# BerkIGuler/AdaFortiTran

Hardware: AMD Instinct MI355X
Metric: OFDM frames/sec (120x14 grid, batch 128) + channel-estimation MSE vs reference (higher is better)
Workload: dtype f32; 1 GPU; C3: AdaFortiTran default config (6 layers, d=128, 4 heads, adaptive tokens), 120x14 grid, pilots 12x2; 128 frames per GPU per step; step = model(pilots_cpu, meta_cpu) through the module surface + device MSE partial; value = SURVEY 8(d)'s metric: H2D of pilots + meta INSIDE the step, output left on the device (= value_h2d_inclusive); the bare engine call on inputs resident in HBM is value_resident;; frames_per_gpu=128, global_batch=128, parallelism=frames sharded over 1 rank(s), lanes=1

## Files before the change

### adafortitran_amd/csrc/aft_api.hip

```cpp
#include <algorithm>
#include <atomic>
#include <cstdlib>
#include <cstdarg>
#include <cstdio>
#include <cstring>
#include <mutex>
#include <string>
#include <vector>

#include "aft_internal.h"

namespace aft {

static thread_local char g_err[512] = "";

void set_error(const char *fmt, ...) {
    va_list ap;
    va_start(ap, fmt);
    vsnprintf(g_err, sizeof(g_err), fmt, ap);
    va_end(ap);
}

int hip_fail(const char *what, hipError_t e) {
    set_error("%s: %s", what, hipGetErrorString(e));
// ... 320 lines not shown
            hit->used = false;
        }
        return nullptr;
    }
    ++hit->in_use;
    hit->tick = ++g_lane_tick;
    return &hit->ls;
}
static void release_lane_streams(LaneStreams *ls) {
    if (ls == nullptr) return;
    std::lock_guard<std::mutex> lock(g_lane_mu);
    for (auto &en : g_lane_cache)
        if (&en.ls == ls) { --en.in_use; return; }
}

enum ChainPos { kChainFirst, kChainMiddle, kChainLast };
static ChainFusion chain_fusion_for(ChainPos pos, const aft_config &c, const WeightsDev &w, const Workspace &ws, float *base) {
    ChainFusion f{};
    f.x_blocked = true;
    if (pos == kChainFirst) {
        f.conv_enhanced = base + ws.conv_enhanced;
        f.tokens6 = c.adaptive ? base + ws.tokens6 : nullptr;
        f.lin1_w = w.lin1_w; f.lin1_b = w.lin1_b; f.pos = w.pos;
    } else if (pos == kChainLast) {
        f.lin2_w = w.lin2_w; f.lin2_b = w.lin2_b; f.out6 = base + ws.out6;
    }
    return f;
}

static int run_encoder(const aft_config &c, const WeightsDev &w, const aft_layer_weights *layers, const Workspace &ws, float *base, float *x,
                       int first_layer, int last_layer, hipStream_t st, bool fused = false, const float *prepacked = nullptr,
                       float *x_pt = nullptr, float *vt2 = nullptr) {
    float *attn = base + ws.attn, *q = base + ws.q, *k = base + ws.k, *vt = base + ws.vt;
    const int rows = ws.planes * ws.tokens;
    const size_t pl = packed_layer_floats(c.model_dim);
    const float *wp = prepacked != nullptr ? prepacked : base + ws.wpack;
    if (prepacked == nullptr)
        STEP("pack_weights", launch_pack_weights(c, layers + first_layer, base + ws.wpack + first_layer * pl, last_layer - first_layer + 1, st));
    const ChainFusion first = chain_fusion_for(kChainFirst, c, w, ws, base), middle = chain_fusion_for(kChainMiddle, c, w, ws, base),
                      last = chain_fusion_for(kChainLast, c, w, ws, base);
    if (fused && x_pt != nullptr && x == base + ws.x && first_layer == 0 && last_layer == c.num_layers - 1 &&
        layer_fused_selected(c, ws.planes / 2)) {
        x = x_pt;
        float *kbuf[2] = {k, attn}, *vbuf[2] = {vt, vt2};
        STEP("chain(qkv, plane tiles)", launch_chain_plane_tiles(c, &layers[0], wp, x, q, kbuf[0], vbuf[0], ws.planes, ws.tokens, ws.tokpad, st, &first));
        for (int l = 0; l <= last_layer; ++l) {
            const bool more = l < last_layer;
            STEP("layer", launch_layer(c, &layers[l], wp + l * pl, more ? &layers[l + 1] : nullptr, more ? wp + (l + 1) * pl : nullptr, x, q,
                                       kbuf[l & 1], vbuf[l & 1], kbuf[(l + 1) & 1], vbuf[(l + 1) & 1], ws.planes, ws.tokens, ws.tokpad, st,
                                       more ? &middle : &last));
        }
        return AFT_OK;
    }
    STEP("chain(qkv)", launch_chain(c, nullptr, nullptr, &layers[first_layer], wp + first_layer * pl, nullptr, x, q, k, vt, rows,
                                    ws.tokens, ws.tokpad, st, fused ? &first : nullptr));
// ... 126 lines not shown
    for (int i = 0; i < kMaxLanes; ++i) {
        frames[i] = i < lp.lanes ? lp.frames[i] : 0;
        offset_bytes[i] = i < lp.lanes ? lp.ws_off[i] * sizeof(float) : 0;
    }
    return AFT_OK;
}

static int forward_lane(const aft_config *cfg, const aft_weights *w, const float *prepacked, const float *pilots, const float *snr,
                        const float *ds, const float *dop, float *out, float *base, int batch, hipStream_t st, float *x_pt, float *vt2) {
    const Workspace ws = plan_workspace(*cfg, batch);
    const bool general = !packed_engine_ok(*cfg);
    const WeightsDev wd = weights_window(*w, 0, cfg->num_layers);
    float *wpack = prepacked != nullptr || general ? nullptr : base + ws.wpack;
    float *lent = x_holds_planes(*cfg, ws) ? base + ws.x : nullptr;
    float *up_planes = prologue_upsample_ok(*cfg, wd) ? lent : nullptr;
    STEP("prologue(adapter + pack_weights + upsampler product)",
         launch_prologue(*cfg, wd, snr, ds, dop, base + ws.tokens6, batch, wpack, pilots, up_planes, st, base + ws.convfrag));
    if (wpack != nullptr && cfg->num_layers > kLayerWindow)
        STEP("pack_weights(layers beyond the prologue's window)",
             launch_pack_weights(*cfg, w->layers + kLayerWindow, wpack + packed_layer_floats(cfg->model_dim) * kLayerWindow,
                                 cfg->num_layers - kLayerWindow, st));
    STEP("upsample", launch_upsample(*cfg, wd, pilots, base + ws.conv_enhanced, batch, st, lent, up_planes != nullptr, base + ws.convfrag));
    const int rc = general ? run_encoder_general(*cfg, wd, w->layers, ws, base, batch, st)
                           : run_encoder(*cfg, wd, w->layers, ws, base, base + ws.x, 0, cfg->num_layers - 1, st, true,
                                         prepacked != nullptr ? prepacked : wpack, x_pt, vt2);
    if (rc != AFT_OK) return rc;
    STEP("tail", launch_tail(*cfg, wd, nullptr, base + ws.conv_enhanced, out, batch, st, base + ws.out6, base + ws.convfrag + kConvFragFloats));
    return AFT_OK;
}

static int forward_impl(const aft_config *cfg, const aft_weights *w, const float *prepacked, const float *pilots,
                        const float *snr, const float *ds, const float *dop, float *out, void *workspace,
                        size_t workspace_bytes, int batch, void *stream) {
    int rc = check_config(cfg);
    if (rc != AFT_OK) return rc;
    AFT_REQUIRE(w && pilots && out && workspace, "NULL pointer argument");
    AFT_REQUIRE(batch > 0, "batch must be positive (got %d)", batch);
    AFT_REQUIRE(batch <= max_batch_of(*cfg), "batch %d exceeds aft_max_batch = %d for this configuration (32-bit buffer "
                "offsets: no workspace region may reach 2 GiB); split the batch", batch, max_batch_of(*cfg));
    AFT_REQUIRE(!cfg->adaptive || (snr && ds && dop), "meta_data is required when channel adaptation is enabled");
// ... 210 lines not shown
    AFT_REQUIRE(batch <= max_batch_of(*cfg), "batch %d exceeds aft_max_batch = %d", batch, max_batch_of(*cfg));
    if (!packed_engine_ok(*cfg)) {
        set_error("aft_profile_kernel_f32 replays the packed engine's kernel classes; this configuration runs the general engine");
        return AFT_ERR_SHAPE;
    }
    const Workspace ws = plan_workspace(*cfg, batch);
    AFT_REQUIRE(workspace_bytes >= ws.total * sizeof(float), "workspace too small");
    const WeightsDev wd = weights_window(*w, 0, cfg->num_layers);
    AFT_REQUIRE(cfg->num_layers >= 2 || which != AFT_KERNEL_CHAIN, "chain profile needs >= 2 layers");
    hipStream_t st = static_cast<hipStream_t>(stream);
    float *base = static_cast<float *>(workspace);
    float *x = base + ws.x, *attn = base + ws.attn, *q = base + ws.q, *k = base + ws.k, *vt = base + ws.vt;
    const int rows = ws.planes * ws.tokens;
    float *lent = x_holds_planes(*cfg, ws) ? x : nullptr;
    const float *wp = base + ws.wpack;
    const ChainFusion first = chain_fusion_for(kChainFirst, *cfg, wd, ws, base), middle = chain_fusion_for(kChainMiddle, *cfg, wd, ws, base),
                      last = chain_fusion_for(kChainLast, *cfg, wd, ws, base);
    hipError_t e = hipSuccess;
    for (int i = 0; i < reps && e == hipSuccess; ++i) {
        switch (which) {
            case AFT_KERNEL_UPSAMPLE:
                AFT_REQUIRE(out != nullptr, "upsample profile needs the pilots pointer in `out`");
                e = launch_upsample(*cfg, wd, out, base + ws.conv_enhanced, batch, st, lent, prologue_upsample_ok(*cfg, wd), base + ws.convfrag);
                break;
            case AFT_KERNEL_EMBED:
                e = launch_embed(*cfg, wd, base + ws.conv_enhanced, cfg->adaptive ? base + ws.tokens6 : nullptr, x, batch, st);
                break;
            case AFT_KERNEL_QKV:
                e = launch_chain(*cfg, nullptr, nullptr, &w->layers[0], wp, nullptr, x, q, k, vt, rows, ws.tokens, ws.tokpad, st, &first);
                break;
            case AFT_KERNEL_ATTENTION:
                e = launch_attention(*cfg, q, k, vt, w->layers[0].in_proj_b, attn, ws.planes, ws.tokens, ws.tokpad, st);
                break;
            case AFT_KERNEL_CHAIN:
                e = launch_chain(*cfg, &w->layers[0], wp, &w->layers[1], wp + packed_layer_floats(cfg->model_dim), attn, x, q, k, vt, rows,
                                 ws.tokens, ws.tokpad, st, &middle);
                break;
            case AFT_KERNEL_CHAIN_LAST:
                e = launch_chain(*cfg, &w->layers[0], wp, nullptr, nullptr, attn, x, q, k, vt, rows, ws.tokens, ws.tokpad, st, &last);
                break;
            case AFT_KERNEL_PROLOGUE: {
                AFT_REQUIRE(out != nullptr, "prologue profile needs the pilots pointer in `out`");
                const float *cond = out + (size_t)batch * cfg->pilot_scs * cfg->pilot_symbols * 2;
                e = launch_prologue(*cfg, wd, cond, cond + batch, cond + 2 * batch, base + ws.tokens6, batch, base + ws.wpack, out,
                                    prologue_upsample_ok(*cfg, wd) && !switch_on(SW_PROLOGUE_NO_UP) ? lent : nullptr, st,
                                    base + ws.convfrag);
                break;
            }
            case AFT_KERNEL_TAIL:
                AFT_REQUIRE(out != nullptr, "tail profile needs an output buffer");
                e = launch_tail(*cfg, wd, nullptr, base + ws.conv_enhanced, out, batch, st, base + ws.out6, base + ws.convfrag + kConvFragFloats);
                break;
            default:
                set_error("unknown kernel id %d", which);
                return AFT_ERR_ARG;
        }
    }
    return e == hipSuccess ? AFT_OK : hip_fail("profile", e);
}

}
// ... 1 lines not shown
```

### adafortitran_amd/csrc/aft_internal.h

```cpp
#pragma once

#include <hip/hip_runtime.h>

#include <cstddef>
#include <cstdint>

#include "../../include/adafortitran_amd.h"
#include "switches.h"
#ifdef AFT_DIAG_STAMPS
#include "stamp_report.h"
#endif

namespace aft {

using f32x2 = __attribute__((ext_vector_type(2))) float;
using f32x4 = __attribute__((ext_vector_type(4))) float;
using f32x16 = __attribute__((ext_vector_type(16))) float;

constexpr int kWave = 64;
constexpr int kHeadDim = 32;
constexpr int kTile = 32;
constexpr int kMaxPatchFeatures = 16;

inline __host__ __device__ int round_up(int v, int m) { return (v + m - 1) / m * m; }
// ... 174 lines not shown
    unsigned long long *dev_ = nullptr;
    std::vector<unsigned long long> host_;
    StampKind kind_;
    long long rows_;
    hipStream_t st_;
};
#endif

constexpr size_t kConvFragFloats = 22 * 64 * 4 + 160;
hipError_t launch_upsample(const aft_config &c, const WeightsDev &w, const float *pilots,
                           float *conv_enhanced, int batch, hipStream_t st, float *scratch_planes = nullptr, bool planes_ready = false,
                           const float *conv_frag = nullptr);
hipError_t launch_adapter(const aft_config &c, const WeightsDev &w, const float *snr, const float *ds,
                          const float *dop, float *tokens6, int batch, hipStream_t st);
bool prologue_upsample_ok(const aft_config &c, const WeightsDev &w);
hipError_t launch_prologue(const aft_config &c, const WeightsDev &w, const float *snr, const float *ds, const float *dop,
                           float *tokens6, int batch, float *packed, const float *pilots, float *up_planes, hipStream_t st,
                           float *conv_frag = nullptr);
hipError_t launch_embed(const aft_config &c, const WeightsDev &w, const float *conv_enhanced,
                        const float *tokens6, float *x, int batch, hipStream_t st);
constexpr int kMaxPatchGeneral = 32;
hipError_t launch_embed_any(const aft_config &c, const WeightsDev &w, const float *conv_enhanced,
                            const float *tokens6, float *x, int batch, hipStream_t st);
struct ChainFusion {
    const float *conv_enhanced = nullptr, *tokens6 = nullptr, *lin1_w = nullptr, *lin1_b = nullptr, *pos = nullptr;
    const float *lin2_w = nullptr, *lin2_b = nullptr;
    float *out6 = nullptr;
    bool x_blocked = false;
};
inline int out6_stride(const aft_config &c) { return round_up(c.patch_scs * c.patch_symbols, 8); }
hipError_t launch_chain(const aft_config &c, const aft_layer_weights *mlp_w, const float *mlp_packed,
                        const aft_layer_weights *qkv_w, const float *qkv_packed, const float *attn, float *x,
                        float *q, float *k, float *vt, int rows, int tokens, int tokpad, hipStream_t st,
                        const ChainFusion *fuse = nullptr);
size_t packed_layer_floats(int d);
bool layer_fused_ok(const aft_config &c);
hipError_t launch_chain_plane_tiles(const aft_config &c, const aft_layer_weights *qkv_w, const float *qkv_packed, float *x, float *q,
                                    float *k, float *vt, int planes, int tokens, int tokpad, hipStream_t st, const ChainFusion *fuse);
hipError_t launch_layer(const aft_config &c, const aft_layer_weights *mlp_w, const float *mlp_packed, const aft_layer_weights *qkv_w,
                        const float *qkv_packed, float *x, float *q, const float *k_in, const float *vt_in, float *k_out, float *vt_out,
                        int planes, int tokens, int tokpad, hipStream_t st, const ChainFusion *fuse);
hipError_t launch_pack_weights(const aft_config &c, const aft_layer_weights *layers, float *packed, int count, hipStream_t st);
// ... 143 lines not shown
```

### adafortitran_amd/csrc/chain_device.h

```cpp
#pragma once
#include "aft_internal.h"
#include "srd.h"
#include "stamps.h"

namespace aft {

template <int D>
struct ChainShape {
    static constexpr int WAVES = D / 32;
    static constexpr int THREADS = 64 * WAVES;
    static constexpr int XB = WAVES * 1024;
    static constexpr int HB = 2 * WAVES * 1024;
    static constexpr int ST = 32 * WAVES * 2;
    static constexpr int PAR = 4 * D;
    static constexpr size_t LDS_BYTES = sizeof(float) * (size_t)(XB + HB + ST + PAR);
};

struct ChainArgs {
    const float *attn;
    float *x;
    const float *wo, *w1, *w2, *wqkv;
    const float *bo, *b1, *b2, *g1, *be1, *g2, *be2;
    const float *bv;
    float *q, *k, *vt;
    int rows, tokens, tokpad, heads;
    int x_blocked;
    const float *lin2_w, *lin2_b;
    float *out6;
    int out6_features, out6_stride;
    const float *emb_conv, *emb_tok6, *emb_w1, *emb_b1, *emb_pos;
    int emb_S, emb_T, emb_p0, emb_p1, emb_K;
    unsigned long long *stamps;
    int tpp;
};

ChainArgs make_chain_args(const aft_config &c, const aft_layer_weights *mlp_w, const float *mlp_packed, const aft_layer_weights *qkv_w,
                          const float *qkv_packed, const float *attn, float *x, float *q, float *k, float *vt, int rows, int tokens,
                          int tokpad, const ChainFusion *fuse);

template <int NT, int PFS>
struct WRing {
    f32x4 b[PFS + 1][NT];
};


template <int NKB, int NT, int PFS, int TS>
// ... 152 lines not shown
    const Srd srd_q = make_srd(a.q), srd_k = make_srd(a.k), srd_vt = make_srd(a.vt);
    const unsigned wo_off = (unsigned)w * W * 1024 + lane * 4, w1_off = (unsigned)(2 * w) * W * 1024 + lane * 4;
    const unsigned w2_off = (unsigned)w * (2 * W) * 1024 + lane * 4;
    const unsigned wq_off = (unsigned)w * W * 1024 + lane * 4;
    const Srd srd_bv = make_srd(a.bv);

    if constexpr (MLP) {
        for (int i = tid; i < D; i += S::THREADS) {
            par[i] = a.g1[i];
            par[D + i] = a.be1[i];
            par[2 * D + i] = a.g2[i];
            par[3 * D + i] = a.be2[i];
        }
        __syncthreads();
    }
    constexpr int kEmbSteps = (kMaxPatchFeatures + 6 + 1) / 2;
    float *emb_w = hb + S::XB;
    int *emb_offs = reinterpret_cast<int *>(emb_w + D * (kMaxPatchFeatures + 6));
    if constexpr (!MLP) {
        if (a.emb_conv != nullptr) {
            const int pk = a.emb_p0 * a.emb_p1;
            for (int i = tid; i < D * a.emb_K; i += S::THREADS) emb_w[i] = a.emb_w1[i];
            for (int k = tid; k < a.emb_K; k += S::THREADS)
                emb_offs[k] = k < pk ? (k / a.emb_p1) * a.emb_T + k % a.emb_p1 : ~(k - pk);
            __syncthreads();
        }
    }
    const int ntiles = (a.rows + 31) / 32;
    const int rounds = (tile_end - first_tile + tile_stride - 1) / tile_stride;
    int round = 0;
#ifndef AFT_CHAIN_PFK
// ... 55 lines not shown
            for (int j = 0; j < 4; ++j) emb_acc0[4 * s + j] = b[j] + ps[j];
        }
#pragma unroll
        for (int st = 0; st < kEmbSteps; ++st) {
            const int k = 2 * st + h;
            emb_bv[st] = 0.f;
            if (k < a.emb_K) {
                const int off = emb_offs[k];
                emb_bv[st] = off >= 0 ? cplane[off] : t6[~off];
            }
        }
    };
    if constexpr (!MLP) {
        if (a.emb_conv != nullptr && first_tile < tile_end) emb_request(first_tile);
    }
    int pending_row0 = -1, pending_valid = 0;
    auto reduce_out6 = [&]() {
        const int P = a.out6_features;
        if (PT ? r < pending_valid : pending_row0 + r < a.rows) {
#pragma unroll
            for (int half = 0; half < 2; ++half) {
                const int f0 = 8 * half + 4 * h;
                if (f0 < P) {
                    f32x4 sum = *reinterpret_cast<const f32x4 *>(hb + lane * 8 + 4 * half);
#pragma unroll
                    for (int u = 1; u < W; ++u) {
                        const f32x4 t = *reinterpret_cast<const f32x4 *>(hb + (u * 64 + lane) * 8 + 4 * half);
                        sum += t;
                    }
#pragma unroll
// ... 43 lines not shown
                   w1_lane = ((PT && MLP ? (unsigned)(2 * w) * W * 1024 : w1_off) + lo_lane) * 4,
                   w2_lane = ((PT && MLP ? (unsigned)w * (2 * W) * 1024 : w2_off) + lo_lane) * 4,
                   wq_lane = ((PT && MLP ? (unsigned)w * W * 1024 : wq_off) + lo_lane) * 4;
    AFT_STAMP(tid == 0, a.stamps, tile, 0);
    AFT_STAMP_WALL(tid == 0, a.stamps, tile, 12);
    AFT_STAMP_VALUE(tid == 0, a.stamps, tile, 14, ((unsigned long long)__builtin_amdgcn_s_getreg((4 << 0) | (0 << 6) | (31 << 11)) << 32) |
                                                      __builtin_amdgcn_s_getreg((20 << 0) | (0 << 6) | (31 << 11)));
#ifndef AFT_CHAIN_PFS
#define AFT_CHAIN_PFS 4
#endif
    constexpr int PFD = AFT_CHAIN_PFS, PFF = (AFT_CHAIN_PFS + 1) / 2, PFQ = (AFT_CHAIN_PFS + 2) / 3;
    WRing<1, PFD> ring_d;
    WRing<2, PFF> ring_ff;
    WRing<3, PFQ> ring_qkv;
    f32x16 cur;
    if constexpr (MLP) {
        f32x16 acc_o[1] = {bias_acc(srd_bo, fb, h)};
        gemm_preload<W, 1, PFD, 1>(ring_d, srd_wo, wo_lane);
        if constexpr (PT) {
            request_x_pt(tile, valid_pt);
        } else {
            request_attn(tile, AHEAD ? PFK : 0, W);
            if (!AHEAD) request_x(tile);
        }
        AFT_STAMP(tid == 0, a.stamps, tile, 1);
        if constexpr (BS)
            gemm_run_bs<W, 1, PFD, 1, 0>(ring_d, srd_wo, wo_lane, acc_o, [&](int kb, int m) { return bs_split(of[kb][2 * m], of[kb][2 * m + 1]); });
        else if constexpr (PT)
            gemm_run<W, 1, PFD, 1, 0>(ring_d, srd_wo, wo_lane, acc_o, [&](int kb, int s) {
                return *reinterpret_cast<const f32x4 *>(hb + S::XB + (kb * 4 + s) * 256 + lane * 4);
// ... 80 lines not shown
            }
        }
        if (store_x && row_ok) {
            if (blocked) {
                const unsigned xblk = ((unsigned)row0 * D + w * 1024 + lane * 4) * 4;
#pragma unroll
                for (int s = 0; s < 4; ++s)
                    srd_store(srd_x, xblk + 1024 * s, f32x4{cur[4 * s], cur[4 * s + 1], cur[4 * s + 2], cur[4 * s + 3]});
            } else {
#pragma unroll
                for (int s = 0; s < 4; ++s)
                    srd_store(srd_x, xrow + 32 * s, f32x4{cur[4 * s], cur[4 * s + 1], cur[4 * s + 2], cur[4 * s + 3]});
            }
        }
    } else {
        gemm_preload<W, 3, PFQ, W>(ring_qkv, srd_wq, wq_lane);
        if (a.emb_conv == nullptr) {
            if (!AHEAD) request_x(tile);
#pragma unroll
            for (int s = 0; s < 4; ++s)
#pragma unroll
                for (int j = 0; j < 4; ++j) cur[4 * s + j] = xres[s][j];
        } else {
            f32x16 acc0 = emb_acc0;
            float av[kEmbSteps];
#pragma unroll
            for (int st = 0; st < kEmbSteps; ++st) {
                const int k = 2 * st + h;
                av[st] = k < a.emb_K ? emb_w[(fb + r) * a.emb_K + k] : 0.f;
            }
#pragma unroll
            for (int st = 0; st < kEmbSteps; ++st)
                if (2 * st < a.emb_K) acc0 = __builtin_amdgcn_mfma_f32_32x32x2f32(av[st], emb_bv[st], acc0, 0, 0, 0);
            cur = acc0;
            if (row_ok) {
                if (blocked) {
                    const unsigned xblk = ((unsigned)row0 * D + w * 1024 + lane * 4) * 4;
#pragma unroll
                    for (int s = 0; s < 4; ++s)
                        srd_store(srd_x, xblk + 1024 * s, f32x4{cur[4 * s], cur[4 * s + 1], cur[4 * s + 2], cur[4 * s + 3]});
                } else {
#pragma unroll
                    for (int s = 0; s < 4; ++s)
                        srd_store(srd_x, xrow + 32 * s, f32x4{cur[4 * s], cur[4 * s + 1], cur[4 * s + 2], cur[4 * s + 3]});
                }
            }
        }
    }

    if constexpr (QKV) {
        const float bias_v = __builtin_bit_cast(float, __builtin_amdgcn_raw_buffer_load_b32(srd_bv, (unsigned)(fb + r) * 4, 0, 0));
        float *xq = xb;
        if constexpr (!MLP) xq = (round & 1) ? hb : xb;
        if constexpr (BS) {
            bs_publish(xq, w, lane, cur);
        } else {
#pragma unroll
            for (int s = 0; s < 4; ++s)
                *reinterpret_cast<f32x4 *>(xq + (w * 4 + s) * 256 + lane * 4) = f32x4{cur[4 * s], cur[4 * s + 1], cur[4 * s + 2], cur[4 * s + 3]};
        }
        __syncthreads();
        AFT_STAMP(tid == 0, a.stamps, tile, 9);
        f32x16 vinit;
#pragma unroll
        for (int e = 0; e < 16; ++e) vinit[e] = bias_v;
        f32x16 acc[3];
        acc[2] = vinit;
        if constexpr (BS) {
            acc[0] = bias_acc(make_srd(a.bv - 2 * D), fb, h);
            auto xq_bs = [&](int kb, int m) { return bs_fetch(xq, kb, m, lane); };
            gemm_run_bs<W, 3, PFQ, W, 0x4, decltype(xq_bs), 0x2>(ring_qkv, srd_wq, wq_lane, acc, xq_bs);
        } else {
            auto xq_frag = [&](int kb, int s) { return *reinterpret_cast<const f32x4 *>(xq + (kb * 4 + s) * 256 + lane * 4); };
            gemm_run<W, 3, PFQ, W, 0x4, decltype(xq_frag), 0x3>(ring_qkv, srd_wq, wq_lane, acc, xq_frag);
        }
        AFT_STAMP(tid == 0, a.stamps, tile, 10);
        if (AHEAD && tile + tile_stride < ntiles) request_tile(tile + tile_stride);
        if constexpr (!MLP) {
            if (a.emb_conv != nullptr && tile + tile_stride < tile_end) emb_request(tile + tile_stride);
        }
        if constexpr (PT) {
            const unsigned ph_base = (unsigned)(plane_pt * a.heads + w) * ((unsigned)a.tokpad * kHeadDim) + (unsigned)qt_pt * 1024;
            if (row_ok) {
#pragma unroll
                for (int s = 0; s < 4; ++s) {
                    srd_store(srd_q, (ph_base + lane * 4 + s * 256) * 4, f32x4{acc[0][4 * s], acc[0][4 * s + 1], acc[0][4 * s + 2], acc[0][4 * s + 3]});
                    srd_store(srd_k, (ph_base + lane * 4 + s * 256) * 4, f32x4{acc[1][4 * s], acc[1][4 * s + 1], acc[1][4 * s + 2], acc[1][4 * s + 3]});
                }
            }
#pragma unroll
// ... 150 lines not shown
```

### adafortitran_amd/csrc/k_chain.hip

```cpp
#include <algorithm>
#include <cstdlib>

#include "chain_device.h"
#include "pack_device.h"

#ifndef AFT_CHAIN_MANY_MAX_D
#define AFT_CHAIN_MANY_MAX_D 96
#endif

namespace aft {

template <int D, int ACT, bool MLP, bool QKV>
__global__ __launch_bounds__(D * 2, D <= 128 ? 3 : 2) void chain_kernel(const ChainArgs a) {
    extern __shared__ __attribute__((aligned(16))) float smem[];
    chain_body<D, ACT, MLP, QKV>(a, smem, threadIdx.x, blockIdx.x, gridDim.x, (a.rows + 31) / 32);
}


template <int D, int ACT, bool MLP, bool QKV>
__global__ __launch_bounds__(D * 2, D <= 128 ? 3 : 2) void chain_split_kernel(const ChainArgs a) {
    extern __shared__ __attribute__((aligned(16))) float smem[];
    chain_body<D, ACT, MLP, QKV, true>(a, smem, threadIdx.x, blockIdx.x, gridDim.x, (a.rows + 31) / 32);
}

// ... 77 lines not shown
ChainArgs make_chain_args(const aft_config &c, const aft_layer_weights *m, const float *m_packed, const aft_layer_weights *qw,
                          const float *q_packed, const float *attn, float *x, float *q, float *k, float *vt, int rows, int tokens,
                          int tokpad, const ChainFusion *fuse) {
    const size_t dd = (size_t)c.model_dim * c.model_dim;
    ChainArgs a{};
    if (fuse != nullptr && fuse->out6 != nullptr && m != nullptr && qw == nullptr) {
        a.lin2_w = fuse->lin2_w; a.lin2_b = fuse->lin2_b; a.out6 = fuse->out6;
        a.out6_features = c.patch_scs * c.patch_symbols;
        a.out6_stride = out6_stride(c);
    }
    if (fuse != nullptr && fuse->conv_enhanced != nullptr && m == nullptr) {
        a.emb_conv = fuse->conv_enhanced; a.emb_tok6 = fuse->tokens6; a.emb_w1 = fuse->lin1_w; a.emb_b1 = fuse->lin1_b;
        a.emb_pos = fuse->pos;
        a.emb_S = c.num_scs; a.emb_T = c.num_symbols; a.emb_p0 = c.patch_scs; a.emb_p1 = c.patch_symbols;
        a.emb_K = c.patch_scs * c.patch_symbols + (fuse->tokens6 ? 6 : 0);
    }
    a.attn = attn;
    a.x = x;
    a.x_blocked = fuse != nullptr && fuse->x_blocked ? 1 : 0;
    if (m != nullptr) {
        a.wo = m_packed + 3 * dd; a.bo = m->out_proj_b;
        a.w1 = m_packed + 4 * dd; a.b1 = m->lin1_b;
        a.w2 = m_packed + 6 * dd; a.b2 = m->lin2_b;
        a.g1 = m->norm1_w; a.be1 = m->norm1_b;
        a.g2 = m->norm2_w; a.be2 = m->norm2_b;
    }
    if (qw != nullptr) {
        a.wqkv = q_packed;
        a.bv = qw->in_proj_b + 2 * c.model_dim;
    }
// ... 37 lines not shown
```

### adafortitran_amd/csrc/k_misc.hip

```cpp
#include <algorithm>

#include "aft_internal.h"
#include "conv_device.h"
#include "pack_device.h"

namespace aft {

struct AdapterArgs {
    const float *cond[3];
    const float *w[3][3], *b[3][3];
    float *tokens6;
    int h0, h1, h2, tokens;
};

__device__ __forceinline__ void adapter_body(const AdapterArgs &a, int b, int e, float *sm) {
    float *a0 = sm, *a1 = sm + a.h0;
    const int tid = threadIdx.x;
    const float x = a.cond[e][b];
    constexpr int kH0Max = 8, kPer2 = 3;
    const bool fast = a.h0 <= kH0Max && a.h1 == 42 && a.h2 <= kPer2 * 256 && a.h1 <= 256;
    if (fast) {
        float w0 = 0.f, b0 = 0.f, w1[kH0Max], b1 = 0.f, b2[kPer2];
        f32x2 w2[kPer2][21];
        if (tid < a.h0) { w0 = a.w[e][0][tid]; b0 = a.b[e][0][tid]; }
// ... 61 lines not shown
    for (int e = 0; e < 3; ++e)
        for (int j = 0; j < 3; ++j) { a.w[e][j] = w.ada_w[e][j]; a.b[e][j] = w.ada_b[e][j]; }
    a.tokens6 = tokens6;
    a.h0 = c.hidden[0]; a.h1 = c.hidden[1]; a.h2 = c.hidden[2];
    a.tokens = (c.num_scs / c.patch_scs) * (c.num_symbols / c.patch_symbols);
    return a;
}

hipError_t launch_adapter(const aft_config &c, const WeightsDev &w, const float *snr, const float *ds,
                          const float *dop, float *tokens6, int batch, hipStream_t st) {
    const AdapterArgs a = adapter_args(c, w, snr, ds, dop, tokens6);
    hipLaunchKernelGGL(adapter_kernel, dim3(batch, 3), dim3(256), sizeof(float) * (a.h0 + a.h1), st, a);
    return hipGetLastError();
}

struct PrologueArgs {
    AdapterArgs ad;
    float *packed;
    const float *pilots;
    float *up_planes;
    int adapter_blocks, pack_blocks, d, num_layers, split;
    int up_bx, npix, pf, nplanes;
    float *conv_frag;
    int frag_blocks;
};

__global__ __launch_bounds__(256) void prologue_kernel(const WeightsDev w, const PrologueArgs a) {
    extern __shared__ __attribute__((aligned(16))) float sm[];
    int blk = blockIdx.x;
    if (blk < a.adapter_blocks) {
        adapter_body(a.ad, blk / 3, blk % 3, sm);
        return;
    }
    blk -= a.adapter_blocks;
    if (blk < a.pack_blocks) {
        pack_weights_vec(w, a.packed, a.d, 0, a.num_layers, a.split, (size_t)blk * 256 + threadIdx.x);
        return;
    }
    blk -= a.pack_blocks;
    if (blk < a.frag_blocks) {
        const int v = blk * 256 + threadIdx.x;
        constexpr int kPerStack = kFragFloats / 4;
        if (v < 2 * kPerStack) {
            const int stack = v / kPerStack, rem = v - stack * kPerStack;
            const float *const *cw = stack ? w.ref_w : w.enh_w;
            const float *const *cb = stack ? w.ref_b : w.enh_b;
            f32x4 o;
            if (rem < kFragQuads * 64) {
                const int quad = rem >> 6, lane = rem & 63;
#pragma unroll
                for (int jj = 0; jj < 4; ++jj) o[jj] = conv_frag16_entry(cw[1], cb[1], cw[2], cb[2], 4 * quad + jj, lane);
// ... 4 lines not shown
            }
            *reinterpret_cast<f32x4 *>(a.conv_frag + (size_t)v * 4) = o;
        }
        return;
    }
    blk -= a.frag_blocks;
    upsample_planes_body(sm, w.up_w, w.up_b, a.pilots, a.up_planes, a.npix, a.pf, a.nplanes, blk % a.up_bx, blk / a.up_bx);
}

bool prologue_upsample_ok(const aft_config &c, const WeightsDev &w) {
    return upsample_planes_ok(w.up_w, c.pilot_scs * c.pilot_symbols);
}

hipError_t launch_prologue(const aft_config &c, const WeightsDev &w, const float *snr, const float *ds, const float *dop,
                           float *tokens6, int batch, float *packed, const float *pilots, float *up_planes, hipStream_t st,
                           float *conv_frag) {
    PrologueArgs a{};
    if (conv_frag != nullptr) {
        a.conv_frag = conv_frag;
        a.frag_blocks = (2 * (kFragFloats / 4) + 255) / 256;
    }
    size_t lds = 0;
    if (c.adaptive) {
        a.ad = adapter_args(c, w, snr, ds, dop, tokens6);
        a.adapter_blocks = 3 * batch;
        lds = sizeof(float) * (a.ad.h0 + a.ad.h1);
    }
    if (packed != nullptr) {
        a.packed = packed; a.d = c.model_dim; a.num_layers = std::min(c.num_layers, kLayerWindow);
        a.split = c.precision == AFT_PRECISION_BF16X3 ? 1 : 0;
        a.pack_blocks = (int)((packed_layer_floats(c.model_dim) * a.num_layers / 4 + 255) / 256);
    }
    int up_blocks = 0;
    if (up_planes != nullptr && prologue_upsample_ok(c, w)) {
        a.pilots = pilots; a.up_planes = up_planes;
        a.npix = c.num_scs * c.num_symbols; a.pf = c.pilot_scs * c.pilot_symbols; a.nplanes = 2 * batch;
        a.up_bx = (a.npix + kUpPix - 1) / kUpPix;
        up_blocks = a.up_bx * ((a.nplanes + kUpPlanes - 1) / kUpPlanes);
        lds = std::max(lds, upsample_planes_lds(a.pf));
    }
    const int blocks = a.adapter_blocks + a.pack_blocks + a.frag_blocks + up_blocks;
    if (blocks == 0) return hipSuccess;
    hipLaunchKernelGGL(prologue_kernel, dim3(blocks), dim3(256), lds, st, w, a);
    return hipGetLastError();
}

struct EmbedArgs {
    const float *conv_enhanced, *tokens6, *w1, *b1, *pos;
    float *x;
    int S, T, p0, p1, tokens, d, din, planes;
};

template <int D, bool ADAPTIVE, int PMAX>
__global__ __launch_bounds__(256) void embed_kernel(const EmbedArgs a) {
    constexpr int PER = D / 32, NF = ADAPTIVE ? PMAX + 6 : PMAX;
    const int tid = threadIdx.x, hw = tid >> 5, lane32 = tid & 31;
// ... 392 lines not shown
```

### adafortitran_amd/csrc/switches.h

```cpp
#pragma once

#define AFT_SWITCHES(X) \
    X(LANES, "AFT_LANES", "1 = never split a forward into lanes; 2 .. 4 = always that many shares (header section \"Lanes\")") \
    X(LAYER_FUSED, "AFT_LAYER_FUSED", "0 = never the one-launch-per-layer sequence (k_layer.hip), 1 = wherever its shape is covered (default: where plane-aligned tiles add no round)") \
    X(PROLOGUE_NO_UP, "AFT_PROLOGUE_NO_UP", "measurement: the profiled prologue launch without the pilot upsampler product") \
    X(CONV_NSPLIT, "AFT_CONV_NSPLIT", "1 | 2 | 4 column ranges per plane in the streaming conv kernels (default: by the batch)") \
    X(CONV_BANDED, "AFT_CONV_BANDED", "the banded conv kernel instead of the column- / row-streaming ones") \
    X(CONV_COLUMN_TILES, "AFT_CONV_COLUMN_TILES", "the column-tiled conv path even where a band plan fits; n > 2 = at least n tiles per plane") \
    X(GEMM_BM, "AFT_GEMM_BM", "64 | 96: row tile of the training GEMM (default: by the shape)") \
    X(EMBED_ANY_OLD, "AFT_EMBED_ANY_OLD", "the general engine's own embedding kernel instead of the training path's") \
    X(EMBED_BWD_GENERIC, "AFT_EMBED_BWD_GENERIC", "the vector embedding backward instead of the MFMA one (model_dim 128)") \
    X(TRAIN_UNFUSED_FWD, "AFT_TRAIN_UNFUSED_FWD", "the launch sequence the fused forward chain of a training layer replaced") \
    X(TRAIN_UNFUSED_BWD, "AFT_TRAIN_UNFUSED_BWD", "the launch sequence the fused backward chain of a training layer replaced") \
    X(TRAIN_ATTN_BWD_SPLIT, "AFT_TRAIN_ATTN_BWD_SPLIT", "the two-pass attention backward instead of the one-pass kernel") \
    X(ATTN_BWD_GROUPS, "AFT_ATTN_BWD_GROUPS", "1 | 4 problems per workgroup of the one-pass attention backward (default: by shape)") \
    X(STAMPS, "AFT_STAMPS", "phase stamps printed on the host: the diag variant only (libaft_hip_diag.so, build.build_diag(): -DAFT_DIAG_STAMPS)") \
    X(ALLOW_COMPOSITE, "AFT_ALLOW_COMPOSITE", "1 = run a configuration the kernels do not cover on the PyTorch-ROCm composite") \
    X(TRAIN_NO_FUSED_ENDS, "AFT_TRAIN_NO_FUSED_ENDS", "training: PyTorch's unfold / cat / add around the dense ends, not fused") \
    X(TRAIN_NO_QKV_CHAIN, "AFT_TRAIN_NO_QKV_CHAIN", "training: every layer runs its own in-projection GEMM (no chained tapes)") \
    X(PRECISION, "AFT_PRECISION", "f32 | bf16x3: the estimators' default hip_precision") \
    X(ENCODER_PATH, "AFT_ENCODER_PATH", "auto | launches | plane: aft_config.encoder_path of every HipEngine (`plane`: retired, runs the launches)")

namespace aft {

// ... 12 lines not shown
```

Baseline: 84990 frames/s.

## Fold layer-0 key/value projection through the embedding into prologue tables

Layer 0's K and V projections are rewritten algebraically: since x0 = W1·features + b1 + pos, K/V = (Wkv·W1)·features + (Wkv·(b1+pos)+bv). The prologue now precomputes per-token bias tables and the folded Wkv·W1 matrices, so the first chain kernel computes K and V with a K-deep MFMA (patch features + 6) instead of a model_dim-deep GEMM, leaving only Q on the full product. This adds work and LDS use to the prologue launch and changes the floating-point summation order for layer-0 keys and values.

```diff
diff --git a/adafortitran_amd/csrc/aft_api.hip b/adafortitran_amd/csrc/aft_api.hip
--- a/adafortitran_amd/csrc/aft_api.hip
+++ b/adafortitran_amd/csrc/aft_api.hip
@@ -358,6 +358,14 @@
         if (&en.ls == ls) { --en.in_use; return; }
 }
 
+static bool l0_fold_selected(const aft_config &c) {
+    return packed_engine_ok(c) && c.precision == AFT_PRECISION_F32 && switch_int(SW_L0_FOLD, 1) != 0;
+}
+static L0Fold l0_fold_at(const aft_config &c, const Workspace &ws, float *base) {
+    float *tables = base + ws.attn;
+    return L0Fold{tables, tables + (size_t)ws.tokpad * c.model_dim, base + ws.wpack + (size_t)c.model_dim * c.model_dim};
+}
+
 enum ChainPos { kChainFirst, kChainMiddle, kChainLast };
 static ChainFusion chain_fusion_for(ChainPos pos, const aft_config &c, const WeightsDev &w, const Workspace &ws, float *base) {
     ChainFusion f{};
@@ -374,15 +382,18 @@
 
 static int run_encoder(const aft_config &c, const WeightsDev &w, const aft_layer_weights *layers, const Workspace &ws, float *base, float *x,
                        int first_layer, int last_layer, hipStream_t st, bool fused = false, const float *prepacked = nullptr,
-                       float *x_pt = nullptr, float *vt2 = nullptr) {
+                       float *x_pt = nullptr, float *vt2 = nullptr, const L0Fold *fold = nullptr) {
     float *attn = base + ws.attn, *q = base + ws.q, *k = base + ws.k, *vt = base + ws.vt;
     const int rows = ws.planes * ws.tokens;
     const size_t pl = packed_layer_floats(c.model_dim);
     const float *wp = prepacked != nullptr ? prepacked : base + ws.wpack;
     if (prepacked == nullptr)
         STEP("pack_weights", launch_pack_weights(c, layers + first_layer, base + ws.wpack + first_layer * pl, last_layer - first_layer + 1, st));
-    const ChainFusion first = chain_fusion_for(kChainFirst, c, w, ws, base), middle = chain_fusion_for(kChainMiddle, c, w, ws, base),
-                      last = chain_fusion_for(kChainLast, c, w, ws, base);
+    ChainFusion first = chain_fusion_for(kChainFirst, c, w, ws, base);
+    const ChainFusion middle = chain_fusion_for(kChainMiddle, c, w, ws, base), last = chain_fusion_for(kChainLast, c, w, ws, base);
+    if (fused && fold != nullptr && first_layer == 0) {
+        first.fold_tk = fold->tk; first.fold_tvt = fold->tvt; first.fold_w = fold->wf;
+    }
     if (fused && x_pt != nullptr && x == base + ws.x && first_layer == 0 && last_layer == c.num_layers - 1 &&
         layer_fused_selected(c, ws.planes / 2)) {
         x = x_pt;
@@ -539,8 +550,11 @@
     float *wpack = prepacked != nullptr || general ? nullptr : base + ws.wpack;
     float *lent = x_holds_planes(*cfg, ws) ? base + ws.x : nullptr;
     float *up_planes = prologue_upsample_ok(*cfg, wd) ? lent : nullptr;
+    const bool fold_on = l0_fold_selected(*cfg);
+    const L0Fold fold = fold_on ? l0_fold_at(*cfg, ws, base) : L0Fold{};
     STEP("prologue(adapter + pack_weights + upsampler product)",
-         launch_prologue(*cfg, wd, snr, ds, dop, base + ws.tokens6, batch, wpack, pilots, up_planes, st, base + ws.convfrag));
+         launch_prologue(*cfg, wd, snr, ds, dop, base + ws.tokens6, batch, wpack, pilots, up_planes, st, base + ws.convfrag,
+                         fold_on ? &fold : nullptr));
     if (wpack != nullptr && cfg->num_layers > kLayerWindow)
         STEP("pack_weights(layers beyond the prologue's window)",
              launch_pack_weights(*cfg, w->layers + kLayerWindow, wpack + packed_layer_floats(cfg->model_dim) * kLayerWindow,
@@ -548,7 +562,7 @@
     STEP("upsample", launch_upsample(*cfg, wd, pilots, base + ws.conv_enhanced, batch, st, lent, up_planes != nullptr, base + ws.convfrag));
     const int rc = general ? run_encoder_general(*cfg, wd, w->layers, ws, base, batch, st)
                            : run_encoder(*cfg, wd, w->layers, ws, base, base + ws.x, 0, cfg->num_layers - 1, st, true,
-                                         prepacked != nullptr ? prepacked : wpack, x_pt, vt2);
+                                         prepacked != nullptr ? prepacked : wpack, x_pt, vt2, fold_on ? &fold : nullptr);
     if (rc != AFT_OK) return rc;
     STEP("tail", launch_tail(*cfg, wd, nullptr, base + ws.conv_enhanced, out, batch, st, base + ws.out6, base + ws.convfrag + kConvFragFloats));
     return AFT_OK;
@@ -789,8 +803,11 @@
     const int rows = ws.planes * ws.tokens;
     float *lent = x_holds_planes(*cfg, ws) ? x : nullptr;
     const float *wp = base + ws.wpack;
-    const ChainFusion first = chain_fusion_for(kChainFirst, *cfg, wd, ws, base), middle = chain_fusion_for(kChainMiddle, *cfg, wd, ws, base),
-                      last = chain_fusion_for(kChainLast, *cfg, wd, ws, base);
+    ChainFusion first = chain_fusion_for(kChainFirst, *cfg, wd, ws, base);
+    const ChainFusion middle = chain_fusion_for(kChainMiddle, *cfg, wd, ws, base), last = chain_fusion_for(kChainLast, *cfg, wd, ws, base);
+    const bool fold_on = l0_fold_selected(*cfg);
+    const L0Fold fold = fold_on ? l0_fold_at(*cfg, ws, base) : L0Fold{};
+    if (fold_on) { first.fold_tk = fold.tk; first.fold_tvt = fold.tvt; first.fold_w = fold.wf; }
     hipError_t e = hipSuccess;
     for (int i = 0; i < reps && e == hipSuccess; ++i) {
         switch (which) {
@@ -819,7 +836,7 @@
                 const float *cond = out + (size_t)batch * cfg->pilot_scs * cfg->pilot_symbols * 2;
                 e = launch_prologue(*cfg, wd, cond, cond + batch, cond + 2 * batch, base + ws.tokens6, batch, base + ws.wpack, out,
                                     prologue_upsample_ok(*cfg, wd) && !switch_on(SW_PROLOGUE_NO_UP) ? lent : nullptr, st,
-                                    base + ws.convfrag);
+                                    base + ws.convfrag, fold_on ? &fold : nullptr);
                 break;
             }
             case AFT_KERNEL_TAIL:
diff --git a/adafortitran_amd/csrc/aft_internal.h b/adafortitran_amd/csrc/aft_internal.h
--- a/adafortitran_amd/csrc/aft_internal.h
+++ b/adafortitran_amd/csrc/aft_internal.h
@@ -212,9 +212,13 @@
 hipError_t launch_adapter(const aft_config &c, const WeightsDev &w, const float *snr, const float *ds,
                           const float *dop, float *tokens6, int batch, hipStream_t st);
 bool prologue_upsample_ok(const aft_config &c, const WeightsDev &w);
+constexpr int kFoldSteps = (kMaxPatchFeatures + 6 + 1) / 2;
+struct L0Fold {
+    float *tk, *tvt, *wf;
+};
 hipError_t launch_prologue(const aft_config &c, const WeightsDev &w, const float *snr, const float *ds, const float *dop,
                            float *tokens6, int batch, float *packed, const float *pilots, float *up_planes, hipStream_t st,
-                           float *conv_frag = nullptr);
+                           float *conv_frag = nullptr, const L0Fold *fold = nullptr);
 hipError_t launch_embed(const aft_config &c, const WeightsDev &w, const float *conv_enhanced,
                         const float *tokens6, float *x, int batch, hipStream_t st);
 constexpr int kMaxPatchGeneral = 32;
@@ -224,6 +228,7 @@
     const float *conv_enhanced = nullptr, *tokens6 = nullptr, *lin1_w = nullptr, *lin1_b = nullptr, *pos = nullptr;
     const float *lin2_w = nullptr, *lin2_b = nullptr;
     float *out6 = nullptr;
+    const float *fold_tk = nullptr, *fold_tvt = nullptr, *fold_w = nullptr;
     bool x_blocked = false;
 };
 inline int out6_stride(const aft_config &c) { return round_up(c.patch_scs * c.patch_symbols, 8); }
diff --git a/adafortitran_amd/csrc/chain_device.h b/adafortitran_amd/csrc/chain_device.h
--- a/adafortitran_amd/csrc/chain_device.h
+++ b/adafortitran_amd/csrc/chain_device.h
@@ -30,6 +30,9 @@
     int out6_features, out6_stride;
     const float *emb_conv, *emb_tok6, *emb_w1, *emb_b1, *emb_pos;
     int emb_S, emb_T, emb_p0, emb_p1, emb_K;
+    const float *fold_tk;
+    const float *fold_tvt;
+    const float *fold_w;
     unsigned long long *stamps;
     int tpp;
 };
@@ -212,7 +215,8 @@
         }
         __syncthreads();
     }
-    constexpr int kEmbSteps = (kMaxPatchFeatures + 6 + 1) / 2;
+    constexpr int kEmbSteps = kFoldSteps;
+    constexpr int kFoldSteps0 = 6;
     float *emb_w = hb + S::XB;
     int *emb_offs = reinterpret_cast<int *>(emb_w + D * (kMaxPatchFeatures + 6));
     if constexpr (!MLP) {
@@ -298,6 +302,9 @@
     if constexpr (!MLP) {
         if (a.emb_conv != nullptr && first_tile < tile_end) emb_request(first_tile);
     }
+    bool fold = false;
+    if constexpr (!MLP && !BS) fold = a.emb_conv != nullptr && a.fold_tk != nullptr;
+    const Srd srd_tk = make_srd(a.fold_tk), srd_tvt = make_srd(a.fold_tvt), srd_fw = make_srd(a.fold_w);
     int pending_row0 = -1, pending_valid = 0;
     auto reduce_out6 = [&]() {
         const int P = a.out6_features;
@@ -371,6 +378,33 @@
     WRing<2, PFF> ring_ff;
     WRing<3, PFQ> ring_qkv;
     f32x16 cur;
+    f32x16 acc[3];
+    auto in_projection = [&]() {
+        const float bias_v = __builtin_bit_cast(float, __builtin_amdgcn_raw_buffer_load_b32(srd_bv, (unsigned)(fb + r) * 4, 0, 0));
+        float *xq = xb;
+        if constexpr (!MLP) xq = (round & 1) ? hb : xb;
+        if constexpr (BS) {
+            bs_publish(xq, w, lane, cur);
+        } else {
+#pragma unroll
+            for (int s = 0; s < 4; ++s)
+                *reinterpret_cast<f32x4 *>(xq + (w * 4 + s) * 256 + lane * 4) = f32x4{cur[4 * s], cur[4 * s + 1], cur[4 * s + 2], cur[4 * s + 3]};
+        }
+        __syncthreads();
+        AFT_STAMP(tid == 0, a.stamps, tile, 9);
+        f32x16 vinit;
+#pragma unroll
+        for (int e = 0; e < 16; ++e) vinit[e] = bias_v;
+        acc[2] = vinit;
+        if constexpr (BS) {
+            acc[0] = bias_acc(make_srd(a.bv - 2 * D), fb, h);
+            auto xq_bs = [&](int kb, int m) { return bs_fetch(xq, kb, m, lane); };
+            gemm_run_bs<W, 3, PFQ, W, 0x4, decltype(xq_bs), 0x2>(ring_qkv, srd_wq, wq_lane, acc, xq_bs);
+        } else {
+            auto xq_frag = [&](int kb, int s) { return *reinterpret_cast<const f32x4 *>(xq + (kb * 4 + s) * 256 + lane * 4); };
+            gemm_run<W, 3, PFQ, W, 0x4, decltype(xq_frag), 0x3>(ring_qkv, srd_wq, wq_lane, acc, xq_frag);
+        }
+    };
     if constexpr (MLP) {
         f32x16 acc_o[1] = {bias_acc(srd_bo, fb, h)};
         gemm_preload<W, 1, PFD, 1>(ring_d, srd_wo, wo_lane);
@@ -481,14 +515,7 @@
             }
         }
     } else {
-        gemm_preload<W, 3, PFQ, W>(ring_qkv, srd_wq, wq_lane);
-        if (a.emb_conv == nullptr) {
-            if (!AHEAD) request_x(tile);
-#pragma unroll
-            for (int s = 0; s < 4; ++s)
-#pragma unroll
-                for (int j = 0; j < 4; ++j) cur[4 * s + j] = xres[s][j];
-        } else {
+        auto embed_x0 = [&]() {
             f32x16 acc0 = emb_acc0;
             float av[kEmbSteps];
 #pragma unroll
@@ -499,48 +526,104 @@
 #pragma unroll
             for (int st = 0; st < kEmbSteps; ++st)
                 if (2 * st < a.emb_K) acc0 = __builtin_amdgcn_mfma_f32_32x32x2f32(av[st], emb_bv[st], acc0, 0, 0, 0);
-            cur = acc0;
+            return acc0;
+        };
+        auto store_x0 = [&](const f32x16 &v) {
             if (row_ok) {
                 if (blocked) {
                     const unsigned xblk = ((unsigned)row0 * D + w * 1024 + lane * 4) * 4;
 #pragma unroll
                     for (int s = 0; s < 4; ++s)
-                        srd_store(srd_x, xblk + 1024 * s, f32x4{cur[4 * s], cur[4 * s + 1], cur[4 * s + 2], cur[4 * s + 3]});
+                        srd_store(srd_x, xblk + 1024 * s, f32x4{v[4 * s], v[4 * s + 1], v[4 * s + 2], v[4 * s + 3]});
                 } else {
 #pragma unroll
                     for (int s = 0; s < 4; ++s)
-                        srd_store(srd_x, xrow + 32 * s, f32x4{cur[4 * s], cur[4 * s + 1], cur[4 * s + 2], cur[4 * s + 3]});
-                }
-            }
+                        srd_store(srd_x, xrow + 32 * s, f32x4{v[4 * s], v[4 * s + 1], v[4 * s + 2], v[4 * s + 3]});
+                }
+            }
+        };
+        if (fold) {
+          if constexpr (!BS) {
+            gemm_preload<W, 1, PFD, 1>(ring_d, srd_wq, wq_lane);
+            const f32x16 x0 = embed_x0();
+            const unsigned tok_k = PT ? (unsigned)min(qt_pt * 32 + r, a.tokens - 1) : (unsigned)grow % (unsigned)a.tokens;
+#pragma unroll
+            for (int s = 0; s < 4; ++s) {
+                const f32x4 t = srd_load(srd_tk, (tok_k * D + fb + 8 * s + 4 * h) * 4);
+#pragma unroll
+                for (int j = 0; j < 4; ++j) acc[1][4 * s + j] = t[j];
+            }
+            const unsigned vrow = (unsigned)(fb + r) * (unsigned)a.tokpad;
+#pragma unroll
+            for (int g = 0; g < 4; ++g) {
+                if constexpr (PT) {
+                    const f32x4 t = srd_load(srd_tvt, (vrow + qt_pt * 32 + 8 * g + 4 * h) * 4);
+#pragma unroll
+                    for (int j = 0; j < 4; ++j) acc[2][4 * g + j] = t[j];
+                } else {
+                    unsigned t = (unsigned)(row0 + 8 * g + 4 * h) % (unsigned)a.tokens;
+#pragma unroll
+                    for (int j = 0; j < 4; ++j) {
+                        acc[2][4 * g + j] = __builtin_bit_cast(float, __builtin_amdgcn_raw_buffer_load_b32(srd_tvt, (vrow + t) * 4, 0, 0));
+                        if (++t >= (unsigned)a.tokens) t = 0;
+                    }
+                }
+            }
+            float fold_wk[kEmbSteps], fold_wv[kEmbSteps];
+            auto frag = [&](int st) {
+                const unsigned fo = ((unsigned)(w * kEmbSteps + st) * 64 + lane + lo) * 4;
+                fold_wk[st] = __builtin_bit_cast(float, __builtin_amdgcn_raw_buffer_load_b32(srd_fw, fo, 0, 0));
+                fold_wv[st] = __builtin_bit_cast(float, __builtin_amdgcn_raw_buffer_load_b32(srd_fw, fo + W * kEmbSteps * 64 * 4, 0, 0));
+            };
+            const bool more_steps = a.emb_K > 2 * kFoldSteps0;
+#pragma unroll
+            for (int st = 0; st < kEmbSteps; ++st) fold_wk[st] = fold_wv[st] = 0.f;
+#pragma unroll
+            for (int st = 0; st < kFoldSteps0; ++st) frag(st);
+            if (more_steps) {
+#pragma unroll
+                for (int st = kFoldSteps0; st < kEmbSteps; ++st) frag(st);
+            }
+            store_x0(x0);
+            float *xq = (round & 1) ? hb : xb;
+#pragma unroll
+            for (int s = 0; s < 4; ++s)
+                *reinterpret_cast<f32x4 *>(xq + (w * 4 + s) * 256 + lane * 4) = f32x4{x0[4 * s], x0[4 * s + 1], x0[4 * s + 2], x0[4 * s + 3]};
+            auto kv_step = [&](int st) {
+                acc[1] = __builtin_amdgcn_mfma_f32_32x32x2f32(fold_wk[st], emb_bv[st], acc[1], 0, 0, 0);
+                acc[2] = __builtin_amdgcn_mfma_f32_32x32x2f32(emb_bv[st], fold_wv[st], acc[2], 0, 0, 0);
+            };
+#pragma unroll
+            for (int st = 0; st < kFoldSteps0; ++st) kv_step(st);
+            if (more_steps) {
+#pragma unroll
+                for (int st = kFoldSteps0; st < kEmbSteps; ++st) kv_step(st);
+            }
+            __syncthreads();
+            AFT_STAMP(tid == 0, a.stamps, tile, 9);
+            f32x16 acc_q[1];
+            auto xq_frag = [&](int kb, int s) { return *reinterpret_cast<const f32x4 *>(xq + (kb * 4 + s) * 256 + lane * 4); };
+            gemm_run<W, 1, PFD, 1, 0, decltype(xq_frag), 0x1>(ring_d, srd_wq, wq_lane, acc_q, xq_frag);
+            acc[0] = acc_q[0];
+          }
+        } else {
+            gemm_preload<W, 3, PFQ, W>(ring_qkv, srd_wq, wq_lane);
+            if (a.emb_conv == nullptr) {
+                if (!AHEAD) request_x(tile);
+#pragma unroll
+                for (int s = 0; s < 4; ++s)
+#pragma unroll
+                    for (int j = 0; j < 4; ++j) cur[4 * s + j] = xres[s][j];
+            } else {
+                cur = embed_x0();
+                store_x0(cur);
+            }
+            if constexpr (QKV) in_projection();
         }
     }
 
     if constexpr (QKV) {
-        const float bias_v = __builtin_bit_cast(float, __builtin_amdgcn_raw_buffer_load_b32(srd_bv, (unsigned)(fb + r) * 4, 0, 0));
-        float *xq = xb;
-        if constexpr (!MLP) xq = (round & 1) ? hb : xb;
-        if constexpr (BS) {
-            bs_publish(xq, w, lane, cur);
-        } else {
-#pragma unroll
-            for (int s = 0; s < 4; ++s)
-                *reinterpret_cast<f32x4 *>(xq + (w * 4 + s) * 256 + lane * 4) = f32x4{cur[4 * s], cur[4 * s + 1], cur[4 * s + 2], cur[4 * s + 3]};
-        }
-        __syncthreads();
-        AFT_STAMP(tid == 0, a.stamps, tile, 9);
-        f32x16 vinit;
-#pragma unroll
-        for (int e = 0; e < 16; ++e) vinit[e] = bias_v;
-        f32x16 acc[3];
-        acc[2] = vinit;
-        if constexpr (BS) {
-            acc[0] = bias_acc(make_srd(a.bv - 2 * D), fb, h);
-            auto xq_bs = [&](int kb, int m) { return bs_fetch(xq, kb, m, lane); };
-            gemm_run_bs<W, 3, PFQ, W, 0x4, decltype(xq_bs), 0x2>(ring_qkv, srd_wq, wq_lane, acc, xq_bs);
-        } else {
-            auto xq_frag = [&](int kb, int s) { return *reinterpret_cast<const f32x4 *>(xq + (kb * 4 + s) * 256 + lane * 4); };
-            gemm_run<W, 3, PFQ, W, 0x4, decltype(xq_frag), 0x3>(ring_qkv, srd_wq, wq_lane, acc, xq_frag);
-        }
+      if constexpr (MLP) in_projection();
         AFT_STAMP(tid == 0, a.stamps, tile, 10);
         if (AHEAD && tile + tile_stride < ntiles) request_tile(tile + tile_stride);
         if constexpr (!MLP) {
diff --git a/adafortitran_amd/csrc/k_chain.hip b/adafortitran_amd/csrc/k_chain.hip
--- a/adafortitran_amd/csrc/k_chain.hip
+++ b/adafortitran_amd/csrc/k_chain.hip
@@ -115,6 +115,9 @@
         a.emb_pos = fuse->pos;
         a.emb_S = c.num_scs; a.emb_T = c.num_symbols; a.emb_p0 = c.patch_scs; a.emb_p1 = c.patch_symbols;
         a.emb_K = c.patch_scs * c.patch_symbols + (fuse->tokens6 ? 6 : 0);
+        if (fuse->fold_tk != nullptr && c.precision == AFT_PRECISION_F32) {
+            a.fold_tk = fuse->fold_tk; a.fold_tvt = fuse->fold_tvt; a.fold_w = fuse->fold_w;
+        }
     }
     a.attn = attn;
     a.x = x;
diff --git a/adafortitran_amd/csrc/k_misc.hip b/adafortitran_amd/csrc/k_misc.hip
--- a/adafortitran_amd/csrc/k_misc.hip
+++ b/adafortitran_amd/csrc/k_misc.hip
@@ -99,6 +99,84 @@
     return hipGetLastError();
 }
 
+
+constexpr int kFoldTok = 2, kFoldChunk = 16;
+struct FoldArgs {
+    const float *wkv, *bv;
+    const float *w1, *b1, *pos;
+    float *tk, *tvt, *wf;
+    int d, K, tokens, tokpad;
+};
+inline size_t fold_tables_lds(int d) { return sizeof(float) * ((size_t)256 * (kFoldChunk + 1) + (size_t)kFoldTok * d); }
+
+__device__ __forceinline__ void fold_tables_body(const FoldArgs &f, int blk, float *sm) {
+    float *sw = sm, *sc = sm + 256 * (kFoldChunk + 1);
+    const int tid = threadIdx.x, chunks = (2 * f.d + 255) / 256;
+    const int t0 = (blk / chunks) * kFoldTok, row0 = (blk % chunks) * 256, row = row0 + tid;
+    for (int i = tid; i < kFoldTok * f.d; i += 256) {
+        const int tt = i / f.d, k = i - tt * f.d, t = t0 + tt;
+        sc[i] = t < f.tokens ? f.b1[k] + f.pos[(size_t)t * f.d + k] : 0.f;
+    }
+    float acc[kFoldTok];
+#pragma unroll
+    for (int tt = 0; tt < kFoldTok; ++tt) acc[tt] = row >= f.d && row < 2 * f.d ? f.bv[row - f.d] : 0.f;
+    constexpr int kPieces = kFoldChunk / 4;
+    f32x4 piece[kPieces];
+    auto request = [&](int kc) {
+#pragma unroll
+        for (int m = 0; m < kPieces; ++m) {
+            const int i = tid + 256 * m, rr = i / kPieces, c4 = (i % kPieces) * 4;
+            piece[m] = f32x4{0.f, 0.f, 0.f, 0.f};
+            if (row0 + rr < 2 * f.d) piece[m] = *reinterpret_cast<const f32x4 *>(f.wkv + (size_t)(row0 + rr) * f.d + kc + c4);
+        }
+    };
+    request(0);
+    for (int kc = 0; kc < f.d; kc += kFoldChunk) {
+        __syncthreads();
+#pragma unroll
+        for (int m = 0; m < kPieces; ++m) {
+            const int i = tid + 256 * m, rr = i / kPieces, c4 = (i % kPieces) * 4;
+#pragma unroll
+            for (int j = 0; j < 4; ++j) sw[rr * (kFoldChunk + 1) + c4 + j] = piece[m][j];
+        }
+        if (kc + kFoldChunk < f.d) request(kc + kFoldChunk);
+        __syncthreads();
+#pragma unroll
+        for (int kk = 0; kk < kFoldChunk; ++kk) {
+            const float wv = sw[tid * (kFoldChunk + 1) + kk];
+#pragma unroll
+            for (int tt = 0; tt < kFoldTok; ++tt) acc[tt] = fmaf(wv, sc[tt * f.d + kc + kk], acc[tt]);
+        }
+    }
+#pragma unroll
+    for (int tt = 0; tt < kFoldTok; ++tt) {
+        const int t = t0 + tt;
+        if (row < f.d) {
+            if (t < f.tokens) f.tk[(size_t)t * f.d + row] = acc[tt];
+        } else if (row < 2 * f.d && t < f.tokpad) {
+            f.tvt[(size_t)(row - f.d) * f.tokpad + t] = t < f.tokens ? acc[tt] : 0.f;
+        }
+    }
+}
+
+__device__ __forceinline__ void fold_matrices_body(const FoldArgs &f, int blk) {
+    const int o = blk * 256 + threadIdx.x, per_part = (f.d / 32) * kFoldSteps * 64;
+    if (o >= 2 * per_part) return;
+    const int part = o / per_part, rem = o - part * per_part;
+    const int wblock = rem / (kFoldSteps * 64), st = rem / 64 % kFoldSteps, lane = rem & 63;
+    const int row = part * f.d + 32 * wblock + (lane & 31), k = 2 * st + (lane >> 5);
+    float acc = 0.f;
+    if (k < f.K) {
+        const float *wr = f.wkv + (size_t)row * f.d;
+        for (int j = 0; j < f.d; j += 4) {
+            const f32x4 wv = *reinterpret_cast<const f32x4 *>(wr + j);
+#pragma unroll
+            for (int jj = 0; jj < 4; ++jj) acc = fmaf(wv[jj], f.w1[(size_t)(j + jj) * f.K + k], acc);
+        }
+    }
+    f.wf[o] = acc;
+}
+
 struct PrologueArgs {
     AdapterArgs ad;
     float *packed;
@@ -108,6 +186,8 @@
     int up_bx, npix, pf, nplanes;
     float *conv_frag;
     int frag_blocks;
+    FoldArgs fold;
+    int fold_table_blocks, fold_matrix_blocks;
 };
 
 __global__ __launch_bounds__(256) void prologue_kernel(const WeightsDev w, const PrologueArgs a) {
@@ -118,8 +198,20 @@
         return;
     }
     blk -= a.adapter_blocks;
+    if (blk < a.fold_table_blocks) {
+        fold_tables_body(a.fold, blk, sm);
+        return;
+    }
+    blk -= a.fold_table_blocks;
+    if (blk < a.fold_matrix_blocks) {
+        fold_matrices_body(a.fold, blk);
+        return;
+    }
+    blk -= a.fold_matrix_blocks;
     if (blk < a.pack_blocks) {
-        pack_weights_vec(w, a.packed, a.d, 0, a.num_layers, a.split, (size_t)blk * 256 + threadIdx.x);
+        const size_t v = (size_t)blk * 256 + threadIdx.x, dd4 = (size_t)a.d * a.d / 4;
+        if (a.fold_table_blocks > 0 && v >= dd4 && v < 3 * dd4) return;
+        pack_weights_vec(w, a.packed, a.d, 0, a.num_layers, a.split, v);
         return;
     }
     blk -= a.pack_blocks;
@@ -154,7 +246,7 @@
 
 hipError_t launch_prologue(const aft_config &c, const WeightsDev &w, const float *snr, const float *ds, const float *dop,
                            float *tokens6, int batch, float *packed, const float *pilots, float *up_planes, hipStream_t st,
-                           float *conv_frag) {
+                           float *conv_frag, const L0Fold *fold) {
     PrologueArgs a{};
     if (conv_frag != nullptr) {
         a.conv_frag = conv_frag;
@@ -179,7 +271,19 @@
         up_blocks = a.up_bx * ((a.nplanes + kUpPlanes - 1) / kUpPlanes);
         lds = std::max(lds, upsample_planes_lds(a.pf));
     }
-    const int blocks = a.adapter_blocks + a.pack_blocks + a.frag_blocks + up_blocks;
+    if (fold != nullptr && fold->tk != nullptr) {
+        FoldArgs &f = a.fold;
+        f.d = c.model_dim; f.K = c.patch_scs * c.patch_symbols + (c.adaptive ? 6 : 0);
+        f.tokens = tokens_of(c); f.tokpad = round_up(f.tokens, kTile);
+        f.wkv = w.layers[0].in_proj_w + (size_t)f.d * f.d; f.bv = w.layers[0].in_proj_b + 2 * f.d;
+        f.w1 = w.lin1_w; f.b1 = w.lin1_b; f.pos = w.pos;
+        f.tk = fold->tk; f.tvt = fold->tvt; f.wf = fold->wf;
+        a.d = c.model_dim;
+        a.fold_table_blocks = (f.tokpad + kFoldTok - 1) / kFoldTok * ((2 * f.d + 255) / 256);
+        a.fold_matrix_blocks = (2 * (f.d / 32) * kFoldSteps * 64 + 255) / 256;
+        lds = std::max(lds, fold_tables_lds(f.d));
+    }
+    const int blocks = a.adapter_blocks + a.fold_table_blocks + a.fold_matrix_blocks + a.pack_blocks + a.frag_blocks + up_blocks;
     if (blocks == 0) return hipSuccess;
     hipLaunchKernelGGL(prologue_kernel, dim3(blocks), dim3(256), lds, st, w, a);
     return hipGetLastError();
diff --git a/adafortitran_amd/csrc/switches.h b/adafortitran_amd/csrc/switches.h
--- a/adafortitran_amd/csrc/switches.h
+++ b/adafortitran_amd/csrc/switches.h
@@ -2,6 +2,7 @@
 
 #define AFT_SWITCHES(X) \
     X(LANES, "AFT_LANES", "1 = never split a forward into lanes; 2 .. 4 = always that many shares (header section \"Lanes\")") \
+    X(L0_FOLD, "AFT_L0_FOLD", "0 = layer 0's keys and values by the model_dim-deep product over x0, not from the input features on the prologue's tables (DESIGN.md 4.1)") \
     X(LAYER_FUSED, "AFT_LAYER_FUSED", "0 = never the one-launch-per-layer sequence (k_layer.hip), 1 = wherever its shape is covered (default: where plane-aligned tiles add no round)") \
     X(PROLOGUE_NO_UP, "AFT_PROLOGUE_NO_UP", "measurement: the profiled prologue launch without the pilot upsampler product") \
     X(CONV_NSPLIT, "AFT_CONV_NSPLIT", "1 | 2 | 4 column ranges per plane in the streaming conv kernels (default: by the batch)") \
```

New measurement: 86280 frames/s, median of 6. 1.02x the previous value.
